# mizeller/OnePose_ST

Measured on AMD Instinct MI355X. Metric: query frames/sec (2D-3D match+PnP) @ 7k x 4800 d256; 1/2/4/8 GPU, higher is better.
Workload: dtype bf16x3 (split-bf16 MFMA, f32 accumulate)

## Files before the change

onepose_st_amd/csrc/prep.hip:

```cpp
#include "tile.h"
#include "crop_pixel.h"

namespace {

__global__ __launch_bounds__(256) void pe_add_transpose_kernel(const float* __restrict__ feat, const float* __restrict__ pe,
                                                               float* __restrict__ out, int Cc, int M) {
    __shared__ float tile[32][33];
    const int tx = threadIdx.x & 31, ty = threadIdx.x >> 5;
    const int m0 = blockIdx.x * 32, c0 = blockIdx.y * 32, b = blockIdx.z;
    const float* f = feat + (size_t)b * Cc * M;
#pragma unroll
    for (int k = 0; k < 4; ++k) {
        const int c = c0 + ty + 8 * k, m = m0 + tx;
        tile[ty + 8 * k][tx] = (c < Cc && m < M) ? f[(size_t)c * M + m] : 0.f;
    }
    __syncthreads();
    float* o = out + (size_t)b * M * Cc;
#pragma unroll
    for (int k = 0; k < 4; ++k) {
        const int m = m0 + ty + 8 * k, c = c0 + tx;
        if (m < M && c < Cc) o[(size_t)m * Cc + c] = tile[tx][ty + 8 * k] + (pe ? pe[(size_t)m * Cc + c] : 0.f);
    }
}

constexpr int KS_THREADS = 1024, KS_WAVES = KS_THREADS / 64;

__global__ __launch_bounds__(KS_THREADS) void kpt_stats_kernel(const float* __restrict__ kpts, long long bs, float* __restrict__ stats, int B, int N) {
    __shared__ float red[KS_WAVES][9];
    const int b = blockIdx.x, tid = threadIdx.x, lane = tid & 63, wave = tid >> 6;
    const float* k = kpts + (size_t)b * bs;
    float s[3] = {0.f, 0.f, 0.f}, mn[3] = {INFINITY, INFINITY, INFINITY}, mx[3] = {-INFINITY, -INFINITY, -INFINITY};
#pragma unroll 4
    for (int i = tid; i < N; i += KS_THREADS) {
#pragma unroll
        for (int d = 0; d < 3; ++d) {
            const float v = k[(size_t)i * 3 + d];
            s[d] += v; mn[d] = fminf(mn[d], v); mx[d] = fmaxf(mx[d], v);
        }
    }
#pragma unroll
    for (int d = 0; d < 3; ++d) {
        s[d] = wave_sum(s[d]);
        mx[d] = wave_max(mx[d]);
        mn[d] = -wave_max(-mn[d]);
    }
    if (lane == 0) {
#pragma unroll
        for (int d = 0; d < 3; ++d) { red[wave][d] = s[d]; red[wave][3 + d] = mn[d]; red[wave][6 + d] = mx[d]; }
    }
    __syncthreads();
    if (tid == 0) {
        float ext = 0.f;
        for (int d = 0; d < 3; ++d) {
            float sum = 0.f, lo = INFINITY, hi = -INFINITY;
            for (int w = 0; w < KS_WAVES; ++w) {
                sum += red[w][d];
                lo = fminf(lo, red[w][3 + d]);
                hi = fmaxf(hi, red[w][6 + d]);
            }
            stats[4 * b + d] = sum / (float)N;
            ext = fmaxf(ext, hi - lo);
        }
        stats[4 * b + 3] = 0.f;
        if (b == 0) stats[4 * B] = ext * 0.6f;
    }
}

constexpr int KD = 256;
constexpr int L0 = 8 + OPHIP_PAD, L1 = 32 + OPHIP_PAD, L2 = 64 + OPHIP_PAD, L3 = 128 + OPHIP_PAD, LO = KD + OPHIP_PAD;

struct KptArgs {
    const float* kpts; long long kbs;
    const float* stats;
    const float* desc; long long dbs;
    const f32x4 *w1, *w2, *w3, *w4;
    const float *b1, *b2, *b3, *b4;
    float* out;
    int B, N;
};

__global__ __launch_bounds__(256) void kpt_encode_kernel(KptArgs p) {
    extern __shared__ __attribute__((aligned(16))) float smem[];
    float* A0 = smem;
    float* A1 = A0 + 32 * L0;
    float* A2 = A1 + 32 * L1;
    float* A3 = A2 + 32 * L2;
    float* Ot = A3 + 32 * L3;
    const int tid = threadIdx.x, lane = tid & 63, wave = tid >> 6;
    const int r = lane & 31, h = lane >> 5;
    const int n0 = blockIdx.x * 32, b = blockIdx.y;
    const float scaling = p.stats[4 * p.B];
    if (tid < 32 * 8) {
        const int row = tid >> 3, d = tid & 7;
        float v = 0.f;
        if (d < 3 && n0 + row < p.N) v = (p.kpts[(size_t)b * p.kbs + (size_t)(n0 + row) * 3 + d] - p.stats[4 * b + d]) / scaling;
        A0[row * L0 + d] = v;
    }
    const float* dsc = p.desc + (size_t)b * p.dbs;
    {
        float dv[KD * 32 / 256];
        const int n = tid & 31, cb = tid >> 5;
        const bool live = n0 + n < p.N;
#pragma unroll
        for (int k = 0; k < KD * 32 / 256; ++k) dv[k] = live ? dsc[(size_t)(cb + 8 * k) * p.N + n0 + n] : 0.f;
#pragma unroll
        for (int k = 0; k < KD * 32 / 256; ++k) Ot[n * LO + cb + 8 * k] = dv[k];
    }
    __syncthreads();
    if (wave == 0) {
        f32x16 acc[1] = {zero16()};
        gemm_lds_x_packed<1, 1>(acc, A0 + r * L0 + 4 * h, 1, p.w1 + lane, 64);
        const float bias = p.b1[r];
#pragma unroll
        for (int reg = 0; reg < 16; ++reg) acc[0][reg] += bias;
        acc_to_lds(acc[0], A1, L1, 0, lane);
    }
    __syncthreads();
    rows_layernorm<32, false, true>(A1, L1, nullptr, nullptr, 1e-5f, wave, lane);
    __syncthreads();
    if (wave < 2) {
        f32x16 acc[1] = {zero16()};
        gemm_lds_x_packed<1>(acc, A1 + r * L1 + 4 * h, 4, p.w2 + (size_t)wave * 4 * 64 + lane, 4 * 64);
        const float bias = p.b2[32 * wave + r];
#pragma unroll
        for (int reg = 0; reg < 16; ++reg) acc[0][reg] += bias;
        acc_to_lds(acc[0], A2, L2, 32 * wave, lane);
    }
    __syncthreads();
    rows_layernorm<64, false, true>(A2, L2, nullptr, nullptr, 1e-5f, wave, lane);
    __syncthreads();
    {
        f32x16 acc[1] = {zero16()};
        gemm_lds_x_packed<1>(acc, A2 + r * L2 + 4 * h, 8, p.w3 + (size_t)wave * 8 * 64 + lane, 8 * 64);
        const float bias = p.b3[32 * wave + r];
#pragma unroll
        for (int reg = 0; reg < 16; ++reg) acc[0][reg] += bias;
        acc_to_lds(acc[0], A3, L3, 32 * wave, lane);
    }
    __syncthreads();
    rows_layernorm<128, false, true>(A3, L3, nullptr, nullptr, 1e-5f, wave, lane);
    __syncthreads();
    {
        f32x16 acc[2] = {zero16(), zero16()};
        gemm_lds_x_packed<2>(acc, A3 + r * L3 + 4 * h, 16, p.w4 + (size_t)(2 * wave) * 16 * 64 + lane, 16 * 64);
#pragma unroll
        for (int t = 0; t < 2; ++t) {
            const int c = 64 * wave + 32 * t + r;
            const float bias = p.b4[c];
#pragma unroll
            for (int reg = 0; reg < 16; ++reg) {
                const int row = acc_row(reg, h);
                Ot[row * LO + c] = Ot[row * LO + c] + (acc[t][reg] + bias);
            }
        }
    }
    __syncthreads();
    float* o = p.out + (size_t)b * p.N * KD;
    for (int rr = 0; rr < 8; ++rr) {
        const int row = 8 * wave + rr;
        if (n0 + row < p.N)
            *reinterpret_cast<f32x4*>(o + (size_t)(n0 + row) * KD + 4 * lane) = *reinterpret_cast<const f32x4*>(Ot + row * LO + 4 * lane);
    }
}

__global__ __launch_bounds__(256) void transpose_cl_kernel(const float* __restrict__ in, float* __restrict__ out, int Cc, int L) {
    __shared__ float tile[32][33];
    const int tx = threadIdx.x & 31, ty = threadIdx.x >> 5;
    const int l0 = blockIdx.x * 32, c0 = blockIdx.y * 32, b = blockIdx.z;
#pragma unroll
    for (int k = 0; k < 4; ++k) {
        const int c = c0 + ty + 8 * k, l = l0 + tx;
        tile[ty + 8 * k][tx] = (c < Cc && l < L) ? in[((size_t)b * Cc + c) * L + l] : 0.f;
    }
    __syncthreads();
#pragma unroll
    for (int k = 0; k < 4; ++k) {
        const int l = l0 + ty + 8 * k, c = c0 + tx;
        if (l < L && c < Cc) out[((size_t)b * L + l) * Cc + c] = tile[tx][ty + 8 * k];
    }
}

__global__ __launch_bounds__(256) void transpose_c128_kernel(const float* __restrict__ in, float* __restrict__ out, int L) {
    __shared__ float tile[128][33];
    const int tid = threadIdx.x, l0 = blockIdx.x * 32, b = blockIdx.y;
    const float* src = in + (size_t)b * 128 * L;
    const int lx = tid & 31, cy = tid >> 5;
#pragma unroll
    for (int k = 0; k < 16; ++k) {
        const int c = cy + 8 * k;
        tile[c][lx] = (l0 + lx < L) ? src[(size_t)c * L + l0 + lx] : 0.f;
    }
    __syncthreads();
    float* dst = out + (size_t)b * L * 128;
    const int p = tid >> 3, q0 = tid & 7;
    if (l0 + p < L) {
#pragma unroll
        for (int m = 0; m < 4; ++m) {
            const int q = q0 + 8 * m;
            f32x4 v = {tile[4 * q][p], tile[4 * q + 1][p], tile[4 * q + 2][p], tile[4 * q + 3][p]};
            *reinterpret_cast<f32x4*>(dst + (size_t)(l0 + p) * 128 + 4 * q) = v;
        }
    }
}

__global__ __launch_bounds__(256) void crop_resize_kernel(const unsigned char* __restrict__ img, int H, int W, int x0, int y0, int wb, int hb,
                                                          int S, float* __restrict__ out) {
    const int X = blockIdx.x * 32 + (threadIdx.x & 31), Y = blockIdx.y * 8 + (threadIdx.x >> 5);
    if (X >= S || Y >= S) return;
    out[(size_t)Y * S + X] = crop_pixel(img, H, W, x0, y0, wb, hb, S, X, Y);
}

}

extern "C" int ophip_crop_resize_gray(const unsigned char* image, int H, int W, int x0, int y0, int x1, int y1, int S, float* out, void* stream) {
    if (!image || !out) return ophip_bad_arg(__func__, "null pointer");
    if (H < 1 || W < 1 || S < 1 || x1 <= x0 || y1 <= y0) return ophip_bad_arg(__func__, "bad sizes (need x1 > x0, y1 > y0)");
    OPHIP_LAUNCH("crop_resize", (hipStream_t)stream, crop_resize_kernel, dim3((S + 31) / 32, (S + 7) / 8), dim3(256), 0, (hipStream_t)stream,
                 image, H, W, x0, y0, x1 - x0, y1 - y0, S, out);
    OPHIP_CHECK_LAUNCH();
    return 0;
}

extern "C" int ophip_pe_add_transpose(const float* feat_nchw, const float* pe_nlc, float* out_nlc, int B, int C, int M, void* stream) {
    if (!feat_nchw || !out_nlc) return ophip_bad_arg(__func__, "null pointer");
    if (B < 1 || C < 1 || M < 1) return ophip_bad_arg(__func__, "bad sizes");
    OPHIP_LAUNCH("pe_add_transpose", (hipStream_t)stream, pe_add_transpose_kernel, dim3((M + 31) / 32, (C + 31) / 32, B), dim3(256), 0, (hipStream_t)stream,
                       feat_nchw, pe_nlc, out_nlc, C, M);
    OPHIP_CHECK_LAUNCH();
    return 0;
}

extern "C" int ophip_transpose_cl(const float* in_bcl, float* out_blc, int B, int C, int L, void* stream) {
    if (!in_bcl || !out_blc) return ophip_bad_arg(__func__, "null pointer");
    if (C == 128) {
        OPHIP_LAUNCH("transpose_cl", (hipStream_t)stream, transpose_c128_kernel, dim3((L + 31) / 32, B), dim3(256), 0, (hipStream_t)stream, in_bcl, out_blc, L);
        OPHIP_CHECK_LAUNCH();
        return 0;
    }
    OPHIP_LAUNCH("transpose_cl", (hipStream_t)stream, transpose_cl_kernel, dim3((L + 31) / 32, (C + 31) / 32, B), dim3(256), 0, (hipStream_t)stream, in_bcl, out_blc, C, L);
    OPHIP_CHECK_LAUNCH();
    return 0;
}

extern "C" int ophip_kpt_encode(const float* keypoints3d, long long kpts_bstride, const float* desc_bcn, long long desc_bstride,
                                const float* wpack, float* stats, float* out_bnc, int B, int N, void* stream_) {
    if (!keypoints3d || !desc_bcn || !wpack || !stats || !out_bnc) return ophip_bad_arg(__func__, "null pointer");
    if (B < 1 || N < 1) return ophip_bad_arg(__func__, "bad sizes");
    hipStream_t stream = (hipStream_t)stream_;
    OPHIP_LAUNCH("kpt_stats", stream, kpt_stats_kernel, dim3(B), dim3(KS_THREADS), 0, stream, keypoints3d, kpts_bstride, stats, B, N);
    OPHIP_CHECK_LAUNCH();
    KptArgs a;
    a.kpts = keypoints3d; a.kbs = kpts_bstride; a.stats = stats; a.desc = desc_bcn; a.dbs = desc_bstride;
    const float* w = wpack;
    a.w1 = reinterpret_cast<const f32x4*>(w); w += 32 * 8;
    a.w2 = reinterpret_cast<const f32x4*>(w); w += 64 * 32;
    a.w3 = reinterpret_cast<const f32x4*>(w); w += 128 * 64;
    a.w4 = reinterpret_cast<const f32x4*>(w); w += 256 * 128;
    a.b1 = w; a.b2 = w + 32; a.b3 = w + 96; a.b4 = w + 224;
    a.out = out_bnc; a.B = B; a.N = N;
    const size_t lds = (size_t)(32 * (L0 + L1 + L2 + L3 + LO)) * sizeof(float);
    if (int rc = ophip_lds_attr(reinterpret_cast<const void*>(kpt_encode_kernel), lds, "hipFuncSetAttribute(kpt_encode)")) return rc;
    OPHIP_LAUNCH("kpt_encode", stream, kpt_encode_kernel, dim3((N + 31) / 32, B), dim3(256), lds, stream, a);
    OPHIP_CHECK_LAUNCH();
    return 0;
}
```

Before: 1527.

## Replace LDS transposes with register quad transposes and retune keypoint prep kernels

```diff
diff --git a/onepose_st_amd/csrc/prep.hip b/onepose_st_amd/csrc/prep.hip
--- a/onepose_st_amd/csrc/prep.hip
+++ b/onepose_st_amd/csrc/prep.hip
@@ -2,6 +2,70 @@
 #include "crop_pixel.h"
 
 namespace {
+
+constexpr int TQ_W = 64;
+
+template <bool VEC, bool ADD>
+__device__ __forceinline__ void transpose_quads(const float* __restrict__ src, const float* __restrict__ addend, float* __restrict__ dst,
+                                                int Cc, int L, int l0, int c0, int lane) {
+    const int g = (lane & 3) | ((lane >> 2) & 4), q = ((lane >> 2) & 3) | ((lane >> 3) & 4);
+    const int c = c0 + 4 * g;
+    if (c >= Cc) return;
+    f32x4 v[2][4];
+#pragma unroll
+    for (int j = 0; j < 2; ++j) {
+        const int l = l0 + 32 * j + 4 * q;
+#pragma unroll
+        for (int k = 0; k < 4; ++k) {
+            const float* row = src + (size_t)(c + k) * L + l;
+            if (VEC) {
+                v[j][k] = (l < L) ? *reinterpret_cast<const f32x4*>(row) : f32x4{0.f, 0.f, 0.f, 0.f};
+            } else {
+#pragma unroll
+                for (int i = 0; i < 4; ++i) v[j][k][i] = (l + i < L) ? row[i] : 0.f;
+            }
+        }
+    }
+    f32x4 a[2][4];
+    if (ADD) {
+#pragma unroll
+        for (int j = 0; j < 2; ++j) {
+#pragma unroll
+            for (int i = 0; i < 4; ++i) {
+                const int l = l0 + 32 * j + 4 * q + i;
+                a[j][i] = (addend && l < L) ? *reinterpret_cast<const f32x4*>(addend + (size_t)l * Cc + c) : f32x4{0.f, 0.f, 0.f, 0.f};
+            }
+        }
+    }
+#pragma unroll
+    for (int j = 0; j < 2; ++j) {
+#pragma unroll
+        for (int i = 0; i < 4; ++i) {
+            const int l = l0 + 32 * j + 4 * q + i;
+            if (l >= L) continue;
+            f32x4 o = {v[j][0][i], v[j][1][i], v[j][2][i], v[j][3][i]};
+            if (ADD) o += a[j][i];
+            *reinterpret_cast<f32x4*>(dst + (size_t)l * Cc + c) = o;
+        }
+    }
+}
+
+template <bool VEC>
+__global__ __launch_bounds__(256) void transpose_cl4_kernel(const float* __restrict__ in, float* __restrict__ out, int Cc, int L) {
+    const int b = blockIdx.z, wave = threadIdx.x >> 6;
+    transpose_quads<VEC, false>(in + (size_t)b * Cc * L, nullptr, out + (size_t)b * L * Cc, Cc, L, blockIdx.x * TQ_W,
+                                blockIdx.y * 128 + 32 * wave, threadIdx.x & 63);
+}
+
+template <bool VEC>
+__global__ __launch_bounds__(64) void pe_add_transpose4_kernel(const float* __restrict__ feat, const float* __restrict__ pe,
+                                                               float* __restrict__ out, int Cc, int M) {
+    const int b = blockIdx.z;
+    transpose_quads<VEC, true>(feat + (size_t)b * Cc * M, pe, out + (size_t)b * M * Cc, Cc, M, blockIdx.x * TQ_W, blockIdx.y * 32,
+                               threadIdx.x);
+}
+
+inline bool aligned16(const void* p) { return (reinterpret_cast<uintptr_t>(p) & 15) == 0; }
 
 __global__ __launch_bounds__(256) void pe_add_transpose_kernel(const float* __restrict__ feat, const float* __restrict__ pe,
                                                                float* __restrict__ out, int Cc, int M) {
@@ -23,30 +87,53 @@
     }
 }
 
-constexpr int KS_THREADS = 1024, KS_WAVES = KS_THREADS / 64;
-
-__global__ __launch_bounds__(KS_THREADS) void kpt_stats_kernel(const float* __restrict__ kpts, long long bs, float* __restrict__ stats, int B, int N) {
+constexpr int KS_THREADS = 1024, KS_WAVES = KS_THREADS / 64, KS_BLOCK = 256, KS_PER = KS_THREADS / KS_BLOCK, KS_STEPS = 4;
+
+__global__ __launch_bounds__(KS_BLOCK) void kpt_stats_kernel(const float* __restrict__ kpts, long long bs, float* __restrict__ stats, int B, int N) {
     __shared__ float red[KS_WAVES][9];
     const int b = blockIdx.x, tid = threadIdx.x, lane = tid & 63, wave = tid >> 6;
     const float* k = kpts + (size_t)b * bs;
-    float s[3] = {0.f, 0.f, 0.f}, mn[3] = {INFINITY, INFINITY, INFINITY}, mx[3] = {-INFINITY, -INFINITY, -INFINITY};
-#pragma unroll 4
-    for (int i = tid; i < N; i += KS_THREADS) {
+    float s[KS_PER][3], mn[KS_PER][3], mx[KS_PER][3];
+#pragma unroll
+    for (int u = 0; u < KS_PER; ++u)
+#pragma unroll
+        for (int d = 0; d < 3; ++d) { s[u][d] = 0.f; mn[u][d] = INFINITY; mx[u][d] = -INFINITY; }
+    for (int base = tid; base < N; base += KS_THREADS * KS_STEPS) {
+        float v[KS_STEPS][KS_PER][3];
+#pragma unroll
+        for (int t = 0; t < KS_STEPS; ++t)
+#pragma unroll
+            for (int u = 0; u < KS_PER; ++u) {
+                const int i = min(base + KS_THREADS * t + KS_BLOCK * u, N - 1);
+#pragma unroll
+                for (int d = 0; d < 3; ++d) v[t][u][d] = k[(size_t)i * 3 + d];
+            }
+#pragma unroll
+        for (int t = 0; t < KS_STEPS; ++t)
+#pragma unroll
+            for (int u = 0; u < KS_PER; ++u) {
+                const bool live = base + KS_THREADS * t + KS_BLOCK * u < N;
+#pragma unroll
+                for (int d = 0; d < 3; ++d) {
+                    s[u][d] += live ? v[t][u][d] : 0.f;
+                    mn[u][d] = live ? fminf(mn[u][d], v[t][u][d]) : mn[u][d];
+                    mx[u][d] = live ? fmaxf(mx[u][d], v[t][u][d]) : mx[u][d];
+                }
+            }
+    }
+#pragma unroll
+    for (int u = 0; u < KS_PER; ++u) {
 #pragma unroll
         for (int d = 0; d < 3; ++d) {
-            const float v = k[(size_t)i * 3 + d];
-            s[d] += v; mn[d] = fminf(mn[d], v); mx[d] = fmaxf(mx[d], v);
-        }
-    }
-#pragma unroll
-    for (int d = 0; d < 3; ++d) {
-        s[d] = wave_sum(s[d]);
-        mx[d] = wave_max(mx[d]);
-        mn[d] = -wave_max(-mn[d]);
-    }
-    if (lane == 0) {
-#pragma unroll
-        for (int d = 0; d < 3; ++d) { red[wave][d] = s[d]; red[wave][3 + d] = mn[d]; red[wave][6 + d] = mx[d]; }
+            s[u][d] = wave_sum(s[u][d]);
+            mx[u][d] = wave_max(mx[u][d]);
+            mn[u][d] = -wave_max(-mn[u][d]);
+        }
+        if (lane == 0) {
+            const int vw = wave + (KS_BLOCK / 64) * u;
+#pragma unroll
+            for (int d = 0; d < 3; ++d) { red[vw][d] = s[u][d]; red[vw][3 + d] = mn[u][d]; red[vw][6 + d] = mx[u][d]; }
+        }
     }
     __syncthreads();
     if (tid == 0) {
@@ -79,7 +166,49 @@
     int B, N;
 };
 
-__global__ __launch_bounds__(256) void kpt_encode_kernel(KptArgs p) {
+constexpr int KE_WAVES = 8, KE_THREADS = 64 * KE_WAVES, KE_RPW = 32 / KE_WAVES;
+
+template <int C>
+__device__ __forceinline__ void kpt_rows_norm(float* img, int ld, int wave, int lane) {
+    constexpr int PER = (C + 63) / 64;
+    float v[KE_RPW][PER], s[KE_RPW], mean[KE_RPW], q[KE_RPW], rstd[KE_RPW];
+#pragma unroll
+    for (int rr = 0; rr < KE_RPW; ++rr) {
+        const float* row = img + (KE_RPW * wave + rr) * ld;
+        s[rr] = 0.f;
+#pragma unroll
+        for (int e = 0; e < PER; ++e) {
+            const int c = lane + 64 * e;
+            v[rr][e] = (c < C) ? row[c] : 0.f;
+            s[rr] += v[rr][e];
+        }
+    }
+#pragma unroll
+    for (int rr = 0; rr < KE_RPW; ++rr) mean[rr] = wave_sum(s[rr]) * (1.0f / C);
+#pragma unroll
+    for (int rr = 0; rr < KE_RPW; ++rr) {
+        q[rr] = 0.f;
+#pragma unroll
+        for (int e = 0; e < PER; ++e) {
+            const int c = lane + 64 * e;
+            const float d = (c < C) ? v[rr][e] - mean[rr] : 0.f;
+            q[rr] += d * d;
+        }
+    }
+#pragma unroll
+    for (int rr = 0; rr < KE_RPW; ++rr) rstd[rr] = 1.0f / sqrtf(wave_sum(q[rr]) * (1.0f / C) + 1e-5f);
+#pragma unroll
+    for (int rr = 0; rr < KE_RPW; ++rr) {
+        float* row = img + (KE_RPW * wave + rr) * ld;
+#pragma unroll
+        for (int e = 0; e < PER; ++e) {
+            const int c = lane + 64 * e;
+            if (c < C) row[c] = fmaxf((v[rr][e] - mean[rr]) * rstd[rr], 0.f);
+        }
+    }
+}
+
+__global__ __launch_bounds__(KE_THREADS) void kpt_encode_kernel(KptArgs p) {
     extern __shared__ __attribute__((aligned(16))) float smem[];
     float* A0 = smem;
     float* A1 = A0 + 32 * L0;
@@ -98,13 +227,14 @@
     }
     const float* dsc = p.desc + (size_t)b * p.dbs;
     {
-        float dv[KD * 32 / 256];
+        constexpr int PER = KD * 32 / KE_THREADS, CB = KE_THREADS / 32;
+        float dv[PER];
         const int n = tid & 31, cb = tid >> 5;
         const bool live = n0 + n < p.N;
 #pragma unroll
-        for (int k = 0; k < KD * 32 / 256; ++k) dv[k] = live ? dsc[(size_t)(cb + 8 * k) * p.N + n0 + n] : 0.f;
-#pragma unroll
-        for (int k = 0; k < KD * 32 / 256; ++k) Ot[n * LO + cb + 8 * k] = dv[k];
+        for (int k = 0; k < PER; ++k) dv[k] = live ? dsc[(size_t)(cb + CB * k) * p.N + n0 + n] : 0.f;
+#pragma unroll
+        for (int k = 0; k < PER; ++k) Ot[n * LO + cb + CB * k] = dv[k];
     }
     __syncthreads();
     if (wave == 0) {
@@ -116,7 +246,7 @@
         acc_to_lds(acc[0], A1, L1, 0, lane);
     }
     __syncthreads();
-    rows_layernorm<32, false, true>(A1, L1, nullptr, nullptr, 1e-5f, wave, lane);
+    kpt_rows_norm<32>(A1, L1, wave, lane);
     __syncthreads();
     if (wave < 2) {
         f32x16 acc[1] = {zero16()};
@@ -127,9 +257,9 @@
         acc_to_lds(acc[0], A2, L2, 32 * wave, lane);
     }
     __syncthreads();
-    rows_layernorm<64, false, true>(A2, L2, nullptr, nullptr, 1e-5f, wave, lane);
-    __syncthreads();
-    {
+    kpt_rows_norm<64>(A2, L2, wave, lane);
+    __syncthreads();
+    if (wave < 4) {
         f32x16 acc[1] = {zero16()};
         gemm_lds_x_packed<1>(acc, A2 + r * L2 + 4 * h, 8, p.w3 + (size_t)wave * 8 * 64 + lane, 8 * 64);
         const float bias = p.b3[32 * wave + r];
@@ -138,26 +268,24 @@
         acc_to_lds(acc[0], A3, L3, 32 * wave, lane);
     }
     __syncthreads();
-    rows_layernorm<128, false, true>(A3, L3, nullptr, nullptr, 1e-5f, wave, lane);
+    kpt_rows_norm<128>(A3, L3, wave, lane);
     __syncthreads();
     {
-        f32x16 acc[2] = {zero16(), zero16()};
-        gemm_lds_x_packed<2>(acc, A3 + r * L3 + 4 * h, 16, p.w4 + (size_t)(2 * wave) * 16 * 64 + lane, 16 * 64);
-#pragma unroll
-        for (int t = 0; t < 2; ++t) {
-            const int c = 64 * wave + 32 * t + r;
-            const float bias = p.b4[c];
-#pragma unroll
-            for (int reg = 0; reg < 16; ++reg) {
-                const int row = acc_row(reg, h);
-                Ot[row * LO + c] = Ot[row * LO + c] + (acc[t][reg] + bias);
-            }
+        f32x16 acc[1] = {zero16()};
+        gemm_lds_x_packed<1>(acc, A3 + r * L3 + 4 * h, 16, p.w4 + (size_t)wave * 16 * 64 + lane, 16 * 64);
+        const int c = 32 * wave + r;
+        const float bias = p.b4[c];
+#pragma unroll
+        for (int reg = 0; reg < 16; ++reg) {
+            const int row = acc_row(reg, h);
+            Ot[row * LO + c] = Ot[row * LO + c] + (acc[0][reg] + bias);
         }
     }
     __syncthreads();
     float* o = p.out + (size_t)b * p.N * KD;
-    for (int rr = 0; rr < 8; ++rr) {
-        const int row = 8 * wave + rr;
+#pragma unroll
+    for (int rr = 0; rr < KE_RPW; ++rr) {
+        const int row = KE_RPW * wave + rr;
         if (n0 + row < p.N)
             *reinterpret_cast<f32x4*>(o + (size_t)(n0 + row) * KD + 4 * lane) = *reinterpret_cast<const f32x4*>(Ot + row * LO + 4 * lane);
     }
@@ -177,29 +305,6 @@
     for (int k = 0; k < 4; ++k) {
         const int l = l0 + ty + 8 * k, c = c0 + tx;
         if (l < L && c < Cc) out[((size_t)b * L + l) * Cc + c] = tile[tx][ty + 8 * k];
-    }
-}
-
-__global__ __launch_bounds__(256) void transpose_c128_kernel(const float* __restrict__ in, float* __restrict__ out, int L) {
-    __shared__ float tile[128][33];
-    const int tid = threadIdx.x, l0 = blockIdx.x * 32, b = blockIdx.y;
-    const float* src = in + (size_t)b * 128 * L;
-    const int lx = tid & 31, cy = tid >> 5;
-#pragma unroll
-    for (int k = 0; k < 16; ++k) {
-        const int c = cy + 8 * k;
-        tile[c][lx] = (l0 + lx < L) ? src[(size_t)c * L + l0 + lx] : 0.f;
-    }
-    __syncthreads();
-    float* dst = out + (size_t)b * L * 128;
-    const int p = tid >> 3, q0 = tid & 7;
-    if (l0 + p < L) {
-#pragma unroll
-        for (int m = 0; m < 4; ++m) {
-            const int q = q0 + 8 * m;
-            f32x4 v = {tile[4 * q][p], tile[4 * q + 1][p], tile[4 * q + 2][p], tile[4 * q + 3][p]};
-            *reinterpret_cast<f32x4*>(dst + (size_t)(l0 + p) * 128 + 4 * q) = v;
-        }
     }
 }
 
@@ -224,6 +329,15 @@
 extern "C" int ophip_pe_add_transpose(const float* feat_nchw, const float* pe_nlc, float* out_nlc, int B, int C, int M, void* stream) {
     if (!feat_nchw || !out_nlc) return ophip_bad_arg(__func__, "null pointer");
     if (B < 1 || C < 1 || M < 1) return ophip_bad_arg(__func__, "bad sizes");
+    if (C % 4 == 0 && aligned16(out_nlc) && aligned16(pe_nlc)) {
+        const dim3 grid((M + TQ_W - 1) / TQ_W, (C + 31) / 32, B);
+        if (M % 4 == 0 && aligned16(feat_nchw))
+            OPHIP_LAUNCH("pe_add_transpose", (hipStream_t)stream, pe_add_transpose4_kernel<true>, grid, dim3(64), 0, (hipStream_t)stream, feat_nchw, pe_nlc, out_nlc, C, M);
+        else
+            OPHIP_LAUNCH("pe_add_transpose", (hipStream_t)stream, pe_add_transpose4_kernel<false>, grid, dim3(64), 0, (hipStream_t)stream, feat_nchw, pe_nlc, out_nlc, C, M);
+        OPHIP_CHECK_LAUNCH();
+        return 0;
+    }
     OPHIP_LAUNCH("pe_add_transpose", (hipStream_t)stream, pe_add_transpose_kernel, dim3((M + 31) / 32, (C + 31) / 32, B), dim3(256), 0, (hipStream_t)stream,
                        feat_nchw, pe_nlc, out_nlc, C, M);
     OPHIP_CHECK_LAUNCH();
@@ -232,8 +346,12 @@
 
 extern "C" int ophip_transpose_cl(const float* in_bcl, float* out_blc, int B, int C, int L, void* stream) {
     if (!in_bcl || !out_blc) return ophip_bad_arg(__func__, "null pointer");
-    if (C == 128) {
-        OPHIP_LAUNCH("transpose_cl", (hipStream_t)stream, transpose_c128_kernel, dim3((L + 31) / 32, B), dim3(256), 0, (hipStream_t)stream, in_bcl, out_blc, L);
+    if (C % 4 == 0 && aligned16(out_blc)) {
+        const dim3 grid((L + TQ_W - 1) / TQ_W, (C + 127) / 128, B);
+        if (L % 4 == 0 && aligned16(in_bcl))
+            OPHIP_LAUNCH("transpose_cl", (hipStream_t)stream, transpose_cl4_kernel<true>, grid, dim3(256), 0, (hipStream_t)stream, in_bcl, out_blc, C, L);
+        else
+            OPHIP_LAUNCH("transpose_cl", (hipStream_t)stream, transpose_cl4_kernel<false>, grid, dim3(256), 0, (hipStream_t)stream, in_bcl, out_blc, C, L);
         OPHIP_CHECK_LAUNCH();
         return 0;
     }
@@ -247,7 +365,7 @@
     if (!keypoints3d || !desc_bcn || !wpack || !stats || !out_bnc) return ophip_bad_arg(__func__, "null pointer");
     if (B < 1 || N < 1) return ophip_bad_arg(__func__, "bad sizes");
     hipStream_t stream = (hipStream_t)stream_;
-    OPHIP_LAUNCH("kpt_stats", stream, kpt_stats_kernel, dim3(B), dim3(KS_THREADS), 0, stream, keypoints3d, kpts_bstride, stats, B, N);
+    OPHIP_LAUNCH("kpt_stats", stream, kpt_stats_kernel, dim3(B), dim3(KS_BLOCK), 0, stream, keypoints3d, kpts_bstride, stats, B, N);
     OPHIP_CHECK_LAUNCH();
     KptArgs a;
     a.kpts = keypoints3d; a.kbs = kpts_bstride; a.stats = stats; a.desc = desc_bcn; a.dbs = desc_bstride;
@@ -260,7 +378,7 @@
     a.out = out_bnc; a.B = B; a.N = N;
     const size_t lds = (size_t)(32 * (L0 + L1 + L2 + L3 + LO)) * sizeof(float);
     if (int rc = ophip_lds_attr(reinterpret_cast<const void*>(kpt_encode_kernel), lds, "hipFuncSetAttribute(kpt_encode)")) return rc;
-    OPHIP_LAUNCH("kpt_encode", stream, kpt_encode_kernel, dim3((N + 31) / 32, B), dim3(256), lds, stream, a);
+    OPHIP_LAUNCH("kpt_encode", stream, kpt_encode_kernel, dim3((N + 31) / 32, B), dim3(KE_THREADS), lds, stream, a);
     OPHIP_CHECK_LAUNCH();
     return 0;
 }
```

After: 1516. No clear change (-0.7%).
